# ducha-aiki/affnet

Measured on NVIDIA H100. Metric: Mpix/s end-to-end HesAffNet(+OriNet)+HardNet, higher is better.
Workload: dtype fp16 operands (fp16 residual planes: AffNet/OriNet weights+activations, HardNet layer 2-3 weights), fp32 accumulate; stencils fp32

## Files before the change

affnet_b200/_lib.py:

```python
import ctypes as C
import os
import subprocess

import torch

HERE = os.path.dirname(os.path.abspath(__file__))
LIB_PATH = os.environ.get("AFFNET_B200_LIB", os.path.join(HERE, "lib", "libaffnet_b200.so"))
AG_MAX_OCTAVES, AG_MAX_LEVELS = 16, 8
NET_AFFNET, NET_ORINET, NET_HARDNET = 0, 1, 2
ENGINE_SIMT, ENGINE_TC, ENGINE_TC_EXACT, ENGINE_TC_FAST, ENGINE_TC2, ENGINE_TC2_BF16 = 0, 1, 2, 3, 4, 5


class AffnetB200Error(RuntimeError):
    pass


class PyramidPlan(C.Structure):
    _fields_ = [
        ("B", C.c_int), ("H", C.c_int), ("W", C.c_int), ("n_octaves", C.c_int), ("n_levels", C.c_int),
        ("h", C.c_int * AG_MAX_OCTAVES), ("w", C.c_int * AG_MAX_OCTAVES),
        ("level_offset", (C.c_longlong * AG_MAX_LEVELS) * AG_MAX_OCTAVES),
        ("total_floats", C.c_longlong),
        ("sigma", (C.c_double * AG_MAX_LEVELS) * AG_MAX_OCTAVES),
        ("blur_sigma", (C.c_double * AG_MAX_LEVELS) * AG_MAX_OCTAVES),
# ... 48 lines not shown
    "ag_detect_ws_carve": (i32, [C.POINTER(PyramidPlan), i32, vp, C.POINTER(DetectWs)]),
    "ag_detect": (i32, [C.POINTER(PyramidPlan), vp, f32, i32, C.POINTER(DetectWs), vp]),
    "ag_detect_level_from_responses": (i32, [vp, vp, vp, i32, i32, C.POINTER(f64), i32, vp, vp, i32, C.POINTER(DetectWs), vp]),
    "ag_select_keypoints": (i32, [C.POINTER(PyramidPlan), C.POINTER(DetectWs), i32, f32, i32, vp, vp, vp, vp, vp, vp]),
    "ag_select_all_workspace_bytes": (sz, [C.POINTER(PyramidPlan), i32]),
    "ag_select_all_keypoints": (i32, [C.POINTER(PyramidPlan), C.POINTER(DetectWs), f32, i32, vp, sz, vp, vp, vp, vp, vp, vp]),
    "ag_select_topk_workspace_bytes": (sz, [C.POINTER(PyramidPlan), i32, i32]),
    "ag_select_topk_keypoints": (i32, [C.POINTER(PyramidPlan), C.POINTER(DetectWs), i32, f32, i32, vp, sz, vp, vp, vp, vp, vp, vp]),
    "ag_extract_patches": (i32, [vp, i32, i32, i32, i32, vp, i32, i32, vp, vp]),
    "ag_extract_patches_pyr": (i32, [C.POINTER(PyramidPlan), vp, vp, vp, vp, vp, i32, i32, vp, vp]),
    "ag_pyramid_level_for_lafs": (i32, [C.POINTER(PyramidPlan), vp, i32, i32, vp, vp, vp]),
    "ag_net_create": (i32, [i32, vp, sz, C.POINTER(vp)]),
    "ag_net_destroy": (None, [vp]),
    "ag_net_blob_floats": (sz, [i32]),
    "ag_net_set_engine": (i32, [vp, i32]),
    "ag_net_get_engine": (i32, [vp]),
    "ag_net_workspace_bytes": (sz, [i32, i32]),
    "ag_mat2_compose": (i32, [vp, vp, vp, i32, vp]),
    "ag_lafs_left_multiply": (i32, [vp, vp, vp, i32, vp]),
    "ag_affnet_forward_raw": (i32, [vp, vp, i32, vp, vp, sz, vp]),
    "ag_orinet_forward_raw": (i32, [vp, vp, i32, vp, vp, sz, vp]),
    "ag_debug_pyramid_mode": (i32, [i32]),
    "ag_debug_tcx_layer": (i32, [vp, vp, i32, i32, vp, vp, sz, vp]),
    "ag_debug_libm": (i32, [vp, vp, i32, vp, vp, vp, vp]),
    "ag_debug_orientation_hist_pyr": (i32, [C.POINTER(PyramidPlan), vp, vp, vp, vp, vp, i32, i32, vp, vp, vp]),
    "ag_debug_baumberg_pyr": (i32, [C.POINTER(PyramidPlan), vp, vp, vp, vp, vp, i32, i32, i32, vp, vp, vp]),
    "ag_affnet_forward": (i32, [vp, vp, i32, vp, i32, vp, vp, sz, vp]),
    "ag_orinet_forward": (i32, [vp, vp, i32, vp, i32, vp, vp, vp, sz, vp]),
    "ag_hardnet_forward": (i32, [vp, vp, i32, vp, i32, vp, vp, sz, vp]),
    "ag_net_forward_pyr": (i32, [vp, C.POINTER(PyramidPlan), vp, vp, vp, vp, vp, i32, vp, vp, sz, vp]),
    "ag_affine_shape_filter": (i32, [vp, vp, vp, vp, vp, vp, i32, i32, i32, i32, vp, vp, vp, vp, vp, vp]),
    "ag_affine_shape_filter_all": (i32, [vp, vp, vp, vp, vp, vp, i32, i32, vp, vp, vp, vp, vp, vp]),
    "ag_affine_shape_filter_topk_workspace_bytes": (sz, [i32, i32]),
    "ag_affine_shape_filter_topk": (i32, [vp, vp, vp, vp, vp, vp, i32, i32, i32, i32, vp, sz, vp, vp, vp, vp, vp, vp]),
    "ag_lafs_apply_rotation": (i32, [vp, vp, i32, vp]),
    "ag_lafs_scale": (i32, [vp, vp, i32, f32, f32, f32, vp]),
    "ag_lafs_to_ell": (i32, [vp, i32, vp, vp]),
    "ag_circular_gauss_kernel": (i32, [i32, f64, vp]),
    "ag_orientation_hist": (i32, [vp, i32, i32, vp, vp, vp]),
    "ag_baumberg_shape": (i32, [vp, i32, i32, vp, vp, vp]),
    "ag_sift_windows": (i32, [i32, vp, vp, C.POINTER(i32), C.POINTER(i32)]),
    "ag_sift_describe": (i32, [vp, i32, i32, f32, vp, vp]),
    "ag_sift_describe_pyr": (i32, [C.POINTER(PyramidPlan), vp, vp, vp, vp, vp, i32, i32, f32, vp, vp]),
    "ag_distance_matrix": (i32, [vp, i32, vp, i32, i32, vp, vp]),
    "ag_match_snn_workspace_bytes": (sz, [i32, i32]),
    "ag_match_snn": (i32, [vp, i32, vp, i32, i32, f32, vp, sz, vp, vp, vp, vp, vp]),
# ... 94 lines not shown
```

affnet_b200/csrc/net_impl.cuh:

```cuda
#pragma once
#include <cuda_fp16.h>

#include <vector>

#include "common.cuh"

#define AG_ENGINE_SIMT 0
#define AG_ENGINE_TC 1
#define AG_ENGINE_TC_EXACT 2
#define AG_ENGINE_TC2 4
#define AG_ENGINE_TC2_BF16 5
#define AG_ENGINE_TC_FAST 3

struct ag_net {
    int kind;
    int engine;
    float* d_w[6];
    float* d_b[6];
    float* d_w1;
    __half* d_wx[6];
    __half* d_all_x;
    __half* d_wx_bf[6];
    __half* d_headh_bf;
    __half* d_wh[6];
// ... 8 lines not shown
};

#include "tc_conv.cuh"

namespace ag {
size_t tc_act_bytes(int kind);
int tc_nsplit(int kind, int layer);
int tc_split_w(int kind);
tc::FirstSrc tc_src_patches(const float* patches);
tc::FirstSrc tc_src_pyramid(const ag_pyramid_plan_t* p, const float* pyr, const float* lafs, const int* oct, const int* lvl, int cap);
int tc_hardnet_forward(const ag_net* net, const tc::FirstSrc& src, int n, int group, const int* count, void* bufA, void* bufB, void* headbuf,
                       float* out, cudaStream_t st);
int tc_trunk_orinet(const ag_net* net, const tc::FirstSrc& src, int n, int group, const int* count, void* bufA, void* bufB, void* feat,
                    cudaStream_t st);
int tc_trunk_affnet(const ag_net* net, const tc::FirstSrc& src, int n, int group, const int* count, void* bufA, void* bufB, void* feat,
                    cudaStream_t st);
int tc_headx_forward(const ag_net* net, const void* feat, int n, int group, const int* count, float* out, float* angle, cudaStream_t st, float* raw = nullptr);
size_t tc_headx_bytes(int n);
void tcx_pack_layer(const float* wf, int ci, int co, int stride, int nsplit, int sw, float scale, std::vector<__half>& out, int bf16 = 0);
int tcx_nsplit(int kind, int layer);
int tcx_split_w(int kind, int layer);
int tcx_stride(int layer);
size_t tcx_act_bytes(int n);
int tcx_trunk_affori(const ag_net* net, const tc::FirstSrc& src, int n, int group, const int* count, void* bufA, void* bufB, void* feat,
                     cudaStream_t st, int upto);
int tcx_trunk_hardnet(const ag_net* net, const tc::FirstSrc& src, int n, int group, const int* count, void* bufA, void* bufB, void* headbuf,
                      cudaStream_t st, int upto, int bf16 = 0);
int tc_hardnet_head(const ag_net* net, const void* headbuf, int n, int group, const int* count, float* out, cudaStream_t st, int bf16 = 0);
}
```

affnet_b200/csrc/nets_simt.cu:

```cuda
#include <math.h>

#include <vector>

#include <cuda_bf16.h>

#include "net_impl.cuh"

namespace ag {

constexpr float BN_EPS = 1e-5f;
constexpr int CNT = 256;

struct LayerCfg {
    int cin, cout, stride, hin;
};
static const LayerCfg kAffCfg[6] = {{1, 16, 1, 32}, {16, 16, 1, 32}, {16, 32, 2, 32}, {32, 32, 1, 16}, {32, 64, 2, 16}, {64, 64, 1, 8}};
static const LayerCfg kHardCfg[6] = {{1, 32, 1, 32}, {32, 32, 1, 32}, {32, 64, 2, 32}, {64, 64, 1, 16}, {64, 128, 2, 16}, {128, 128, 1, 8}};

}

namespace ag {

template <int CIN, int COUT, int HIN, int STRIDE, int CT, int CK, bool NORM>
__global__ void __launch_bounds__(CNT) conv3x3_kernel(const float* __restrict__ in, float* __restrict__ out,
// ... 507 lines not shown
    if ((rc = launch_conv<32, 32, 32, 1, 32, 32, false>(a, b, net->d_w[1], net->d_b[1], n, group, count, st))) return rc;
    if ((rc = launch_conv<32, 64, 32, 2, 64, 32, false>(b, a, net->d_w[2], net->d_b[2], n, group, count, st))) return rc;
    if ((rc = launch_conv<64, 64, 16, 1, 64, 32, false>(a, b, net->d_w[3], net->d_b[3], n, group, count, st))) return rc;
    if ((rc = launch_conv<64, 128, 16, 2, 128, 16, false>(b, a, net->d_w[4], net->d_b[4], n, group, count, st))) return rc;
    if ((rc = launch_conv<128, 128, 8, 1, 128, 16, false>(a, b, net->d_w[5], net->d_b[5], n, group, count, st))) return rc;
    return AG_OK;
}

static int run_trunk(const ag_net* net, const float* patches, const tc::FirstSrc* pyr_src, int n, int group, const int* count, float* a,
                     float* b, float** feat, cudaStream_t st) {
    if (net->engine != AG_ENGINE_SIMT) {
        const tc::FirstSrc src = pyr_src ? *pyr_src : tc_src_patches(patches);
        char* base = (char*)a;
        const size_t total = 2 * (size_t)((char*)b - (char*)a);
        const size_t act = net->engine == AG_ENGINE_TC2 ? align_up(tcx_act_bytes(n), 256)
                                                        : align_up((size_t)n * tc_act_bytes(net->engine == AG_ENGINE_TC_FAST ? net->kind : AG_NET_ORINET), 256);
        const size_t fbytes = tc_headx_bytes(n);
        if (2 * act + fbytes > total) { set_error("tensor-core workspace too small"); return AG_ERR_CAPACITY; }
        void* bufA = base;
        void* bufB = base + act;
        b = (float*)(base + 2 * act);
        *feat = b;
        if (net->kind == AG_NET_HARDNET) { set_error("HardNet tensor-core path has its own entry"); return AG_ERR_INVALID; }
        if (net->engine == AG_ENGINE_TC2) return tcx_trunk_affori(net, src, n, group, count, bufA, bufB, b, st, 6);
        if (net->engine != AG_ENGINE_TC_FAST) return tc_trunk_orinet(net, src, n, group, count, bufA, bufB, b, st);
        return tc_trunk_affnet(net, src, n, group, count, bufA, bufB, b, st);
    }
    *feat = b;
    if (patches == nullptr) { set_error("the fp32 SIMT engine needs materialised patches"); return AG_ERR_INVALID; }
    return net->kind == AG_NET_HARDNET ? trunk_hardnet(net, patches, n, group, count, a, b, st)
                                       : trunk_affnet(net, patches, n, group, count, a, b, st);
}

static int split_ws(int kind, int n, void* d_ws, size_t ws_bytes, float** a, float** b) {
    const size_t need = ag_net_workspace_bytes(kind, n);
    if (d_ws == nullptr || ws_bytes < need) {
        set_error("net forward: workspace of %zu bytes needed, %zu given", need, ws_bytes);
        return AG_ERR_CAPACITY;
    }
    *a = (float*)d_ws;
    *b = (float*)((char*)d_ws + need / 2);
    return AG_OK;
}

}

extern "C" {
// ... 105 lines not shown
```

affnet_b200/csrc/nets_tcx.cu:

```cuda
#include <stdlib.h>
#include <string.h>

#include <vector>

#include <cuda_bf16.h>

#include "net_impl.cuh"
#include "tcx_conv.cuh"
#include "tcx_first.cuh"

namespace ag {
namespace tcx {

static int num_sms() {
    static int n = 0;
    if (n == 0) {
        int dev = 0;
        cudaGetDevice(&dev);
        cudaDeviceGetAttribute(&n, cudaDevAttrMultiProcessorCount, dev);
        if (n <= 0) n = 132;
    }
    return n;
}

static int ensure_smem_attr(const void* func, int bytes, bool* configured, const char* what) {
    int dev = 0;
    cudaGetDevice(&dev);
    dev &= 63;
    if (configured[dev]) return AG_OK;
    int rc = check_cuda(cudaFuncSetAttribute(func, cudaFuncAttributeMaxDynamicSharedMemorySize, bytes), what);
    if (rc == AG_OK) configured[dev] = true;
    return rc;
// ... 4 lines not shown
    using Cfg = XCfg<CIN, COUT, H, STRIDE, NSPLIT, STAGES, OUT, SA, SW, OSA>;
    auto kern = tcx_conv_kernel<CIN, COUT, H, STRIDE, NSPLIT, STAGES, OUT, SA, SW, OSA, BF, MC, PPS>;
    static bool configured[64] = {};
    int rc = ensure_smem_attr((const void*)kern, (int)Cfg::SMEM, configured, "tcx_conv smem attr");
    if (rc != AG_OK) return rc;
    XArgs a;
    a.in = (const __half*)in; a.out = out; a.wpk = w; a.bias = b; a.inv_scale = inv_scale; a.n = n; a.group = group; a.count = count;
    const int units = Cfg::In::PAIR ? (n + 1) / 2 : n;
    int gx = num_sms() / NSPLIT;
    if (gx > units) gx = units;
    if (gx < 1) gx = 1;
    if (MC) {
        cudaLaunchConfig_t cfg;
        memset(&cfg, 0, sizeof(cfg));
        cfg.gridDim = dim3(gx, NSPLIT); cfg.blockDim = dim3(Cfg::THREADS); cfg.dynamicSmemBytes = Cfg::SMEM; cfg.stream = st;
        cudaLaunchAttribute attr[1];
        attr[0].id = cudaLaunchAttributeClusterDimension;
        attr[0].val.clusterDim.x = 1; attr[0].val.clusterDim.y = 2; attr[0].val.clusterDim.z = 1;
        cfg.attrs = attr; cfg.numAttrs = 1;
        rc = check_cuda(cudaLaunchKernelEx(&cfg, kern, a), "tcx_conv cluster launch");
        if (rc != AG_OK) return rc;
    } else
        kern<<<dim3(gx, NSPLIT), Cfg::THREADS, Cfg::SMEM, st>>>(a);
    AG_CHECK_LAUNCH("tcx_conv_kernel");
    return AG_OK;
}

template <int C1, int COUT, int SA, int SW, int OSA, int BF = 0, int L3 = 0>
static int launch_first(void* out, const __half* w, const float* b, float inv_scale, int n, int group, const int* count, cudaStream_t st, const FirstSrc& src,
                        void* out3 = nullptr, const __half* w3 = nullptr, const float* b3 = nullptr, float inv_scale3 = 0.f) {
    using Cfg = XFirstCfg<C1, COUT, SA, SW, OSA, L3>;
    auto kern = tcx_first_kernel<C1, COUT, SA, SW, OSA, BF, L3>;
    static bool configured[64] = {};
    int rc = ensure_smem_attr((const void*)kern, (int)Cfg::SMEM, configured, "tcx_first smem attr");
    if (rc != AG_OK) return rc;
    XArgs a;
    a.in = nullptr; a.out = out; a.wpk = w; a.bias = b; a.inv_scale = inv_scale; a.n = n; a.group = group; a.count = count;
    XArgs a3 = a;
    a3.out = out3; a3.wpk = w3; a3.bias = b3; a3.inv_scale = inv_scale3;
    int gx = num_sms();
    if (gx > n) gx = n;
    if (gx < 1) gx = 1;
    kern<<<gx, Cfg::THREADS, Cfg::SMEM, st>>>(a, src, a3);
    AG_CHECK_LAUNCH("tcx_first_kernel");
    return AG_OK;
}
// ... 69 lines not shown

int tcx_nsplit(int kind, int layer) { return (kind == AG_NET_HARDNET && layer >= 4) ? 2 : 1; }
#ifndef AG_HARD_SW2
#define AG_HARD_SW2 1
#endif
#ifndef AG_HARD_SW3
#define AG_HARD_SW3 1
#endif
#ifndef AG_HARD_SW4
#define AG_HARD_SW4 0
#endif
int tcx_split_w(int kind, int layer) { return kind == AG_NET_HARDNET ? (layer == 1 ? AG_HARD_SW2 : layer == 2 ? AG_HARD_SW3 : layer == 3 ? AG_HARD_SW4 : 0) : 1; }
int tcx_stride(int layer) { return (layer == 2 || layer == 4) ? 2 : 1; }

size_t tcx_act_bytes(int n) { return (size_t)(n + 1) * 65536; }

#ifndef AG_HARD_MC5
#define AG_HARD_MC5 1
#endif
#ifndef AG_HARD_MC6
#define AG_HARD_MC6 0
#endif
int tcx_trunk_affori(const ag_net* net, const tc::FirstSrc& src0, int n, int group, const int* count, void* bufA, void* bufB, void* feat,
                     cudaStream_t st, int upto) {
    using namespace tcx;
    tc::FirstSrc src = src0;
    src.w1 = net->d_w1; src.b1 = net->d_b[0]; src.w1_inv = net->w_inv_scale[0]; src.w1_scale = 1.0f / net->w_inv_scale[0];
    int rc;
    if (upto <= 2) return launch_first<16, 16, 1, 1, 1>(bufB, net->d_wx[1], net->d_b[1], net->w_inv_scale[1], n, group, count, st, src);
    if ((rc = launch_first<16, 16, 1, 1, 1, 0, 1>(nullptr, net->d_wx[1], net->d_b[1], net->w_inv_scale[1], n, group, count, st, src,
                                                   bufA, net->d_wx[2], net->d_b[2], net->w_inv_scale[2]))) return rc;
    if (upto <= 3) return AG_OK;
    if ((rc = launch_conv<32, 32, 16, 1, 1, 4, L_S2_8P, 1, 1, 1>(bufA, bufB, net->d_wx[3], net->d_b[3], net->w_inv_scale[3], n, group, count, st))) return rc;
    if (upto <= 4) return AG_OK;
    if ((rc = launch_conv<32, 64, 16, 2, 1, 2, L_S1_8P, 1, 1, 1>(bufB, bufA, net->d_wx[4], net->d_b[4], net->w_inv_scale[4], n, group, count, st))) return rc;
    if (upto <= 5) return AG_OK;
    return launch_conv<64, 64, 8, 1, 1, 2, L_HEAD, 1, 1, 1, 0, 0, 1>(bufA, feat, net->d_wx[5], net->d_b[5], net->w_inv_scale[5], n, group, count, st);
}

template <int BF>
static int trunk_hardnet_t(const ag_net* net, const tc::FirstSrc& src0, int n, int group, const int* count, void* bufA, void* bufB, void* headbuf,
                           cudaStream_t st, int upto) {
    using namespace tcx;
    tc::FirstSrc src = src0;
    src.w1 = net->d_w1; src.b1 = net->d_b[0]; src.w1_inv = net->w_inv_scale[0]; src.w1_scale = 1.0f / net->w_inv_scale[0];
    __half* const* wx = BF ? net->d_wx_bf : net->d_wx;
    int rc;
    if ((rc = launch_first<32, 32, 0, AG_HARD_SW2, 0, BF>(bufB, wx[1], net->d_b[1], net->w_inv_scale[1], n, group, count, st, src))) return rc;
    if (upto <= 2) return AG_OK;
    if ((rc = launch_conv<32, 64, 32, 2, 1, 2, L_S1_16, 0, AG_HARD_SW3, 0, BF>(bufB, bufA, wx[2], net->d_b[2], net->w_inv_scale[2], n, group, count, st))) return rc;
    if (upto <= 3) return AG_OK;
    if ((rc = launch_conv<64, 64, 16, 1, 1, 2, L_S2_8P, 0, AG_HARD_SW4, 0, BF>(bufA, bufB, wx[3], net->d_b[3], net->w_inv_scale[3], n, group, count, st))) return rc;
    if (upto <= 4) return AG_OK;
    if ((rc = launch_conv<64, 128, 16, 2, 2, 2, L_S1_8P, 0, 0, 0, BF, AG_HARD_MC5, 1>(bufB, bufA, wx[4], net->d_b[4], net->w_inv_scale[4], n, group, count, st))) return rc;
    if (upto <= 5) return AG_OK;
    return launch_conv<128, 128, 8, 1, 2, 2, L_HEAD, 0, 0, 0, BF, AG_HARD_MC6, 1>(bufA, headbuf, wx[5], net->d_b[5], net->w_inv_scale[5], n, group, count, st);
}

int tcx_trunk_hardnet(const ag_net* net, const tc::FirstSrc& src0, int n, int group, const int* count, void* bufA, void* bufB, void* headbuf,
                      cudaStream_t st, int upto, int bf16) {
    return bf16 ? trunk_hardnet_t<1>(net, src0, n, group, count, bufA, bufB, headbuf, st, upto)
                : trunk_hardnet_t<0>(net, src0, n, group, count, bufA, bufB, headbuf, st, upto);
}

}

using namespace ag;

extern "C" {

int ag_debug_tcx_layer(const ag_net_t* net, const float* d_patches, int n, int upto, float* d_out, void* d_ws, size_t ws_bytes, void* stream) {
    AG_REQUIRE(net && d_patches && d_out && d_ws, "NULL argument");
    AG_REQUIRE(upto >= 2 && upto <= 6 && n >= 1, "layer out of range");
    const size_t act = align_up(tcx_act_bytes(n), 256);
    AG_REQUIRE(ws_bytes >= ag_net_workspace_bytes(net->kind, n), "workspace too small");
    cudaStream_t st = (cudaStream_t)stream;
    char* base = (char*)d_ws;
    const tc::FirstSrc src = tc_src_patches(d_patches);
    const bool hard = net->kind == AG_NET_HARDNET;
    const int bf = hard && net->engine == AG_ENGINE_TC2_BF16;
    int rc = hard ? tcx_trunk_hardnet(net, src, n, n, nullptr, base, base + act, base + 2 * act, st, upto, bf)
                  : tcx_trunk_affori(net, src, n, n, nullptr, base, base + act, base + 2 * act, st, upto);
    if (rc) return rc;
    const int lay = upto == 2 ? tcx::L_S2_16 : upto == 3 ? tcx::L_S1_16 : upto == 4 ? tcx::L_S2_8P : upto == 5 ? tcx::L_S1_8P : tcx::L_HEAD;
    const int H = upto == 2 ? 32 : (upto <= 4 ? 16 : 8);
    const int Cb = hard ? 32 : 16;
    const int C = upto == 2 ? Cb : (upto <= 4 ? 2 * Cb : 4 * Cb);
    const void* buf = upto == 6 ? base + 2 * act : (upto == 2 || upto == 4) ? base + act : base;
    const int osa = hard ? 0 : 1;
    tcx::tcx_decode_kernel<<<296, 256, 0, st>>>((const __half*)buf, lay, C, osa, H, n, bf, d_out);
    AG_CHECK_LAUNCH("tcx_decode_kernel");
    return AG_OK;
}

#ifdef AG_FIRST_TIMELINE
int ag_first_timeline_read(unsigned long long* host, int* dims, int reset) {
    constexpr size_t n = (size_t)tcx::TL_LAUNCHES * tcx::TL_CTAS * 16 * tcx::TL_STATES;
    if (dims) { dims[0] = tcx::TL_LAUNCHES; dims[1] = tcx::TL_CTAS; dims[2] = tcx::TL_STATES; }
    cudaDeviceSynchronize();
    if (host) {
        const int rc = check_cuda(cudaMemcpyFromSymbol(host, tcx::g_first_tl, n * 8), "timeline read");
        if (rc != AG_OK) return rc;
    }
    if (reset) {
        static unsigned long long zeros[n];
        static int zl[tcx::TL_CTAS];
        int rc = check_cuda(cudaMemcpyToSymbol(tcx::g_first_tl, zeros, sizeof(zeros)), "timeline reset");
        if (rc == AG_OK) rc = check_cuda(cudaMemcpyToSymbol(tcx::g_first_tl_launch, zl, sizeof(zl)), "timeline reset");
        return rc;
    }
    return AG_OK;
}
#endif
// ... 24 lines not shown
```

affnet_b200/csrc/tcx_conv.cuh:

```cuda
#pragma once
#include <cuda_bf16.h>

#include "tc_conv.cuh"

#ifndef AG_CONV_PINGPONG
#define AG_CONV_PINGPONG 1
#endif

namespace ag {
namespace tcx {

using namespace ag::tc;

constexpr int XORDER = 5;

enum { CT_TOTAL, CT_WAIT_FULL, CT_TURN, CT_ISSUE, CT_MMA_WAIT, CT_EPILOGUE, CT_WG_BAR, CT_WAIT_EMPTY, CT_OTHER, CT_STATES };
#ifdef AG_CONV_TIMELINE
constexpr int CT_CTAS = 4, CT_LAUNCHES = 16, CT_EVENTS = 2048;
__device__ unsigned long long g_conv_tl[CT_LAUNCHES][CT_CTAS][9][CT_STATES];
__device__ unsigned long long g_conv_ev[CT_LAUNCHES][2][CT_EVENTS][3];
__device__ int g_conv_tl_launch[CT_CTAS];
struct ConvTimeline {
    unsigned long long t[CT_STATES];
    long long start, mark;
    int slot, warp, n_ev;
    __device__ static void claim(int* s_slot) {
        if (threadIdx.x == 0)
            *s_slot = (blockIdx.y == 0 && blockIdx.x < CT_CTAS) ? min(atomicAdd(&g_conv_tl_launch[blockIdx.x], 1), CT_LAUNCHES) : CT_LAUNCHES;
    }
    __device__ void init(const int* s_slot) {
        for (int i = 0; i < CT_STATES; i++) t[i] = 0;
        slot = *s_slot; warp = threadIdx.x >> 5; n_ev = 0;
        start = mark = clock64();
    }
    __device__ void lap(int state) { const long long now = clock64(); t[state] += (unsigned long long)(now - mark); mark = now; }
    __device__ void event(int k) {
        if (blockIdx.x == 0 && slot < CT_LAUNCHES && (threadIdx.x & 127) == 0 && n_ev < CT_EVENTS) g_conv_ev[slot][warp >> 2][n_ev][k] = (unsigned long long)mark;
        if (k == 2) n_ev++;
    }
    __device__ void finish() {
        t[CT_TOTAL] = (unsigned long long)(clock64() - start);
        if ((threadIdx.x & 31) == 0 && slot < CT_LAUNCHES)
            for (int i = 0; i < CT_STATES; i++) g_conv_tl[slot][blockIdx.x][warp][i] = t[i];
    }
};
#else
struct ConvTimeline {
    __device__ static void claim(int*) {}
    __device__ void init(const int*) {}
    __device__ void lap(int) {}
    __device__ void event(int) {}
    __device__ void finish() {}
};
#endif

enum XLayout { L_S2_16 = 0, L_S1_16 = 1, L_S2_8P = 2, L_S1_8P = 3, L_HEAD = 4 };

__device__ __forceinline__ void bulk_g2s_mc(void* dst, const void* src, uint32_t bytes, uint64_t* bar, uint16_t mask) {
    asm volatile("cp.async.bulk.shared::cluster.global.mbarrier::complete_tx::bytes.multicast::cluster [%0], [%1], %2, [%3], %4;" ::"r"(smem_u32(dst)),
                 "l"(src), "r"(bytes), "r"(smem_u32(bar)), "h"(mask)
                 : "memory");
}
__device__ __forceinline__ void mbar_arrive_cluster(uint64_t* bar, uint32_t cta) {
    asm volatile("{\n .reg .b32 ra;\n mapa.shared::cluster.u32 ra, %0, %1;\n mbarrier.arrive.release.cta.shared::cluster.b64 _, [ra];\n}\n" ::"r"(smem_u32(bar)), "r"(cta)
                 : "memory");
}
__device__ __forceinline__ void cluster_sync() {
    asm volatile("barrier.cluster.arrive.release.aligned;\n barrier.cluster.wait.acquire.aligned;" ::: "memory");
}

template <int BF>
__device__ __forceinline__ uint32_t pack2(float a, float b) {
    if (BF) { const __nv_bfloat162 h = __floats2bfloat162_rn(a, b); return *reinterpret_cast<const uint32_t*>(&h); }
    const __half2 h = __floats2half2_rn(a, b);
// ... 124 lines not shown
            constexpr int PL = In::PLANE;
            const int py = (dy == 1) ? 0 : 1, ro = (dy == 0) ? 0 : 1;
#pragma unroll
            for (int j = 0; j < KC / 2; j++) {
                const uint32_t blk = w_base + (uint32_t)((dy * (KC / 2) + j) * 2 * (Cfg::NRO + Cfg::NRE));
                const uint32_t bo_hi = (blk & 0x3FFFu) | ((uint32_t)Cfg::NRO << 16), bo_lo = ((blk + 2 * NT) & 0x3FFFu) | ((uint32_t)Cfg::NRO << 16);
                const uint32_t be = blk + 2 * Cfg::NRO;
                const uint32_t be_hi = (be & 0x3FFFu) | ((uint32_t)Cfg::NRE << 16), be_lo = ((be + NT) & 0x3FFFu) | ((uint32_t)Cfg::NRE << 16);
                const uint32_t ao = a_t + (uint32_t)((py * 2 + 1) * PL + ro * RW);
                const uint32_t ao_hi = ((ao + (uint32_t)(2 * j * GS)) & 0x3FFFu) | LBO_A, ao_lo = ((ao + (uint32_t)((KC + 2 * j) * GS)) & 0x3FFFu) | LBO_A;
                Wgmma<2 * NT, BF>::mma(d, desc64(ao_hi), desc64(bo_hi), (dy | j) != 0);
                if (SW) Wgmma<2 * NT, BF>::mma(d, desc64(ao_hi), desc64(bo_lo), 1);
                if (SA) Wgmma<2 * NT, BF>::mma(d, desc64(ao_lo), desc64(bo_hi), 1);
                const uint32_t ae = a_t + (uint32_t)((py * 2 + 0) * PL + ro * RW);
                const uint32_t ae_hi = ((ae + (uint32_t)(2 * j * GS)) & 0x3FFFu) | LBO_A, ae_lo = ((ae + (uint32_t)((KC + 2 * j) * GS)) & 0x3FFFu) | LBO_A;
                Wgmma<NT, BF>::mma(d + NT, desc64(ae_hi), desc64(be_hi), (dy | j) != 0);
                if (SW) Wgmma<NT, BF>::mma(d + NT, desc64(ae_hi), desc64(be_lo), 1);
                if (SA) Wgmma<NT, BF>::mma(d + NT, desc64(ae_lo), desc64(be_hi), 1);
            }
        }
    }
    wgmma_commit();
}
template <class Cfg, int BF>
__device__ __forceinline__ void xconv_block_epilogue(const float* d, const XArgs& a, const float* s_bias, int u, int b, int split, int wq, int lane) {
    using In = typename Cfg::In;
    constexpr int NT = Cfg::NT, HOUT = Cfg::HOUT, W = In::W, PAIR = In::PAIR, COUT = Cfg::CO, OUT = Cfg::OUTL, OSA = Cfg::SPLIT_O;
    unsigned char* obase[2];
    bool ok[2];
    size_t lo_off = 0;
    const int i = lane >> 2, xi = PAIR ? (i & 3) : i;
    const bool has_l0 = xi > 0, has_r1 = xi < W / 2 - 1;
    static_assert(W == 16 || PAIR, "neighbour-paired row groups: 16 pixels, or 8 of each patch of a pair");
#pragma unroll
    for (int h = 0; h < 2; h++) {
        const int y = b * 4 + wq, x = 2 * xi + h, pi = PAIR ? 2 * u + (i >> 2) : u;
        ok[h] = xpatch_valid(a, pi);
        if (OUT == L_HEAD) {
            obase[h] = reinterpret_cast<unsigned char*>(a.out) + (((size_t)(pi >> 7) * (HOUT * HOUT * COUT / 8) + (size_t)(y * HOUT + x) * (COUT / 8)) * 128 + (pi & 127)) * 16;
            lo_off = (size_t)((a.n + 127) >> 7) * (HOUT * HOUT * COUT / 8) * 128 * 16;
        } else {
            const int ou = layout_pair(OUT) ? (pi >> 1) : pi;
            obase[h] = reinterpret_cast<unsigned char*>(a.out) + (size_t)ou * Cfg::UNIT_OUT_BYTES + (size_t)layout_slot(OUT, y, x, pi & 1) * 16;
            lo_off = (size_t)(COUT / 8) * layout_slots(OUT) * 16;
        }
    }
#pragma unroll
    for (int j = 0; j < NT / 8; j++) {
        const int c = j * 8 + 2 * (lane & 3);
        float v[2][2];
#pragma unroll
        for (int e = 0; e < 2; e++) {
            const float c00 = d[4 * j + e], c01 = d[4 * j + 2 + e];
            const float c10 = d[4 * (j + NT / 8) + e], c11 = d[4 * (j + NT / 8) + 2 + e];
            const float c20 = d[4 * (j + 2 * NT / 8) + e], c21 = d[4 * (j + 2 * NT / 8) + 2 + e];
            const float l0 = frag_left_even(c01, lane);
            float acc0, acc1;
            if (Cfg::STRD == 1) {
                const float r1 = frag_right_odd(c20, lane);
                const float t0 = c21 + c10, t1 = has_r1 ? r1 + c11 : c11;
                acc0 = has_l0 ? l0 + t0 : t0;
                acc1 = c00 + t1;
            } else {
                const float t0 = c10 + c20, t1 = c11 + c21;
                acc0 = has_l0 ? l0 + t0 : t0;
                acc1 = c00 + t1;
            }
            v[0][e] = fmaxf(fmaf(acc0, a.inv_scale, s_bias[c + e]), 0.f);
            v[1][e] = fmaxf(fmaf(acc1, a.inv_scale, s_bias[c + e]), 0.f);
        }
        const int ch = split * NT + c;
        const size_t goff = ((OUT == L_HEAD) ? (size_t)(ch / 8) * 128 * 16 : (size_t)(ch / 8) * layout_slots(OUT) * 16) + (ch & 7) * 2;
#pragma unroll
        for (int h = 0; h < 2; h++) {
            if (!ok[h]) continue;
            uint32_t hi, lo;
            split_pack2<OSA, BF>(v[h][0], v[h][1], hi, lo);
            *reinterpret_cast<uint32_t*>(obase[h] + goff) = hi;
            if (OSA) *reinterpret_cast<uint32_t*>(obase[h] + lo_off + goff) = lo;
        }
    }
}

template <int CIN, int COUT, int H, int STRIDE, int NSPLIT, int STAGES, int OUT, int SA, int SW, int OSA, int BF = 0, int MC = 0, int PPS = 0>
__global__ void __launch_bounds__(288, 1) tcx_conv_kernel(const XArgs a) {
    static_assert(MC == 0 || NSPLIT == 2, "multicast pairs the two channel-split CTAs");
    using Cfg = XCfg<CIN, COUT, H, STRIDE, NSPLIT, STAGES, OUT, SA, SW, OSA>;
    using In = typename Cfg::In;
    constexpr int ACCW = Cfg::ACCW, BLOCKS = Cfg::BLOCKS, GS = Cfg::GS, RW = In::RW;
    constexpr int PAIR = In::PAIR;
    constexpr bool PP = AG_CONV_PINGPONG && PPS;
    extern __shared__ __align__(1024) unsigned char smem[];
    uint64_t* full = reinterpret_cast<uint64_t*>(smem);
    uint64_t* empty = full + STAGES;
    uint64_t* wbar = empty + STAGES;
// ... 109 lines not shown
```

include/affnet_b200.h:

```cpp
#ifndef AFFNET_B200_H
#define AFFNET_B200_H

#include <stddef.h>
#include <stdint.h>

#ifdef __cplusplus
extern "C" {
#endif

#define AG_OK 0
#define AG_ERR_INVALID -1
#define AG_ERR_CUDA -2
#define AG_ERR_CAPACITY -3
#define AG_ERR_NO_DEVICE -4

#define AG_MAX_OCTAVES 16
#define AG_MAX_LEVELS 8

const char* ag_last_error(void);
int ag_abi_version(void);

int ag_prof_begin(void* stream);
int ag_prof_end(void);
int ag_prof_get(int i, const char** name, float* ms);
// ... 58 lines not shown

int ag_extract_patches(const float* d_img, int C, int h, int w, int per_patch_img, const float* d_lafs, int n,
                       int PS, float* d_out, void* stream);

int ag_extract_patches_pyr(const ag_pyramid_plan_t* plan, const float* d_pyr, const float* d_lafs, const int* d_oct,
                           const int* d_lvl, const int* d_count, int cap, int PS, float* d_out, void* stream);

int ag_pyramid_level_for_lafs(const ag_pyramid_plan_t* plan, const float* d_dlafs, int n, int PS, int* d_oct,
                              int* d_lvl, void* stream);

#define AG_NET_AFFNET 0
#define AG_NET_ORINET 1
#define AG_NET_HARDNET 2

typedef struct ag_net ag_net_t;

int ag_net_create(int kind, const float* h_blob, size_t n_floats, ag_net_t** out);
void ag_net_destroy(ag_net_t* net);
size_t ag_net_blob_floats(int kind);
int ag_net_set_engine(ag_net_t* net, int engine);
int ag_net_get_engine(const ag_net_t* net);
int ag_debug_pyramid_mode(int fused);
int ag_debug_tcx_layer(const ag_net_t* net, const float* d_patches, int n, int upto, float* d_out, void* d_ws, size_t ws_bytes, void* stream);
int ag_debug_libm(const float* d_y, const float* d_x, int n, float* d_atan2, float* d_cos, float* d_sin, void* stream);
int ag_debug_orientation_hist_pyr(const ag_pyramid_plan_t* plan, const float* d_pyr, const float* d_lafs, const int* d_oct, const int* d_lvl,
                                  const int* d_count, int cap, int PS, const float* h_gk, float* d_R, void* stream);
int ag_debug_baumberg_pyr(const ag_pyramid_plan_t* plan, const float* d_pyr, const float* d_lafs, const int* d_oct, const int* d_lvl,
                          const int* d_count, int cap, int PS, int iters, const float* h_gk, float* d_A, void* stream);
size_t ag_net_workspace_bytes(int kind, int n);

int ag_affnet_forward(const ag_net_t* net, const float* d_patches, int n, const int* d_count, int group, float* d_out,
                      void* d_ws, size_t ws_bytes, void* stream);
int ag_orinet_forward(const ag_net_t* net, const float* d_patches, int n, const int* d_count, int group, float* d_out,
                      float* d_angle, void* d_ws, size_t ws_bytes, void* stream);
int ag_hardnet_forward(const ag_net_t* net, const float* d_patches, int n, const int* d_count, int group, float* d_out,
                       void* d_ws, size_t ws_bytes, void* stream);

int ag_affnet_forward_raw(const ag_net_t* net, const float* d_patches, int n, float* d_raw, void* d_ws, size_t ws_bytes, void* stream);
int ag_orinet_forward_raw(const ag_net_t* net, const float* d_patches, int n, float* d_raw, void* d_ws, size_t ws_bytes, void* stream);
int ag_net_forward_pyr(const ag_net_t* net, const ag_pyramid_plan_t* plan, const float* d_pyr, const float* d_lafs, const int* d_oct,
                       const int* d_lvl, const int* d_count, int cap, float* d_out, void* d_ws, size_t ws_bytes, void* stream);

int ag_affine_shape_filter(const float* d_A, const float* d_resp, const float* d_lafs, const int* d_oct,
                           const int* d_lvl, const int* d_count_in, int B, int cap, int num_features, int out_cap,
                           float* d_resp_out, float* d_lafs_out, int* d_oct_out, int* d_lvl_out, int* d_count_out,
                           void* stream);
// ... 97 lines not shown
```

Measured before the change: 682.4.

## Fuse AffNet/OriNet conv layers 4 and 5 into one persistent wgmma kernel

Adds a persistent kernel that computes trunk layer 4 for a pair of patches and writes its output straight into shared memory in the layout layer 5 reads, then runs layer 5 from smem. This removes one launch and the global-memory round trip of the layer-4 activations for AffNet/OriNet on the TC2 engine. It is enabled by default through a compile-time flag and changes which buffer holds the layer-5 output. In exchange it uses fewer pipeline stages and serialises layer 5 behind both layer-4 patches, which can lower overlap. A debug entry point is added to compare the fused and unfused paths.

```diff
diff --git a/affnet_b200/_lib.py b/affnet_b200/_lib.py
--- a/affnet_b200/_lib.py
+++ b/affnet_b200/_lib.py
@@ -94,6 +94,7 @@
     "ag_orinet_forward_raw": (i32, [vp, vp, i32, vp, vp, sz, vp]),
     "ag_debug_pyramid_mode": (i32, [i32]),
     "ag_debug_tcx_layer": (i32, [vp, vp, i32, i32, vp, vp, sz, vp]),
+    "ag_debug_tcx_l5": (i32, [vp, vp, i32, i32, vp, i32, vp, vp, sz, vp]),
     "ag_debug_libm": (i32, [vp, vp, i32, vp, vp, vp, vp]),
     "ag_debug_orientation_hist_pyr": (i32, [C.POINTER(PyramidPlan), vp, vp, vp, vp, vp, i32, i32, vp, vp, vp]),
     "ag_debug_baumberg_pyr": (i32, [C.POINTER(PyramidPlan), vp, vp, vp, vp, vp, i32, i32, i32, vp, vp, vp]),
diff --git a/affnet_b200/csrc/net_impl.cuh b/affnet_b200/csrc/net_impl.cuh
--- a/affnet_b200/csrc/net_impl.cuh
+++ b/affnet_b200/csrc/net_impl.cuh
@@ -54,8 +54,11 @@
 int tcx_split_w(int kind, int layer);
 int tcx_stride(int layer);
 size_t tcx_act_bytes(int n);
+#ifndef AG_AFFORI_FUSE45
+#define AG_AFFORI_FUSE45 1
+#endif
 int tcx_trunk_affori(const ag_net* net, const tc::FirstSrc& src, int n, int group, const int* count, void* bufA, void* bufB, void* feat,
-                     cudaStream_t st, int upto);
+                     cudaStream_t st, int upto, int fuse45);
 int tcx_trunk_hardnet(const ag_net* net, const tc::FirstSrc& src, int n, int group, const int* count, void* bufA, void* bufB, void* headbuf,
                       cudaStream_t st, int upto, int bf16 = 0);
 int tc_hardnet_head(const ag_net* net, const void* headbuf, int n, int group, const int* count, float* out, cudaStream_t st, int bf16 = 0);
diff --git a/affnet_b200/csrc/nets_simt.cu b/affnet_b200/csrc/nets_simt.cu
--- a/affnet_b200/csrc/nets_simt.cu
+++ b/affnet_b200/csrc/nets_simt.cu
@@ -553,7 +553,7 @@
         b = (float*)(base + 2 * act);
         *feat = b;
         if (net->kind == AG_NET_HARDNET) { set_error("HardNet tensor-core path has its own entry"); return AG_ERR_INVALID; }
-        if (net->engine == AG_ENGINE_TC2) return tcx_trunk_affori(net, src, n, group, count, bufA, bufB, b, st, 6);
+        if (net->engine == AG_ENGINE_TC2) return tcx_trunk_affori(net, src, n, group, count, bufA, bufB, b, st, 6, AG_AFFORI_FUSE45);
         if (net->engine != AG_ENGINE_TC_FAST) return tc_trunk_orinet(net, src, n, group, count, bufA, bufB, b, st);
         return tc_trunk_affnet(net, src, n, group, count, bufA, bufB, b, st);
     }
diff --git a/affnet_b200/csrc/nets_tcx.cu b/affnet_b200/csrc/nets_tcx.cu
--- a/affnet_b200/csrc/nets_tcx.cu
+++ b/affnet_b200/csrc/nets_tcx.cu
@@ -8,6 +8,7 @@
 #include "net_impl.cuh"
 #include "tcx_conv.cuh"
 #include "tcx_first.cuh"
+#include "tcx_l45.cuh"
 
 namespace ag {
 namespace tcx {
@@ -58,6 +59,27 @@
         if (rc != AG_OK) return rc;
     } else
         kern<<<dim3(gx, NSPLIT), Cfg::THREADS, Cfg::SMEM, st>>>(a);
+    AG_CHECK_LAUNCH("tcx_conv_kernel");
+    return AG_OK;
+}
+
+using XL4 = XCfg<32, 32, 16, 1, 1, 1, L_S2_8P, 1, 1, 1>;
+using XL5 = XCfg<32, 64, 16, 2, 1, 1, L_S1_8P, 1, 1, 1>;
+static int launch_l45(const void* in, void* out, const __half* w4, const float* b4, float inv4, const __half* w5, const float* b5, float inv5, int n,
+                      int group, const int* count, cudaStream_t st) {
+    using Cfg = XL45Cfg<XL4, XL5>;
+    auto kern = tcx_l45_kernel<XL4, XL5>;
+    static bool configured[64] = {};
+    int rc = ensure_smem_attr((const void*)kern, (int)Cfg::SMEM, configured, "tcx_l45 smem attr");
+    if (rc != AG_OK) return rc;
+    XArgs a4, a5;
+    a4.in = (const __half*)in; a4.out = nullptr; a4.wpk = w4; a4.bias = b4; a4.inv_scale = inv4; a4.n = n; a4.group = group; a4.count = count;
+    a5 = a4;
+    a5.in = nullptr; a5.out = out; a5.wpk = w5; a5.bias = b5; a5.inv_scale = inv5;
+    int gx = num_sms();
+    if (gx > (n + 1) / 2) gx = (n + 1) / 2;
+    if (gx < 1) gx = 1;
+    kern<<<gx, Cfg::THREADS, Cfg::SMEM, st>>>(a4, a5);
     AG_CHECK_LAUNCH("tcx_conv_kernel");
     return AG_OK;
 }
@@ -173,7 +195,7 @@
 #define AG_HARD_MC6 0
 #endif
 int tcx_trunk_affori(const ag_net* net, const tc::FirstSrc& src0, int n, int group, const int* count, void* bufA, void* bufB, void* feat,
-                     cudaStream_t st, int upto) {
+                     cudaStream_t st, int upto, int fuse45) {
     using namespace tcx;
     tc::FirstSrc src = src0;
     src.w1 = net->d_w1; src.b1 = net->d_b[0]; src.w1_inv = net->w_inv_scale[0]; src.w1_scale = 1.0f / net->w_inv_scale[0];
@@ -182,11 +204,18 @@
     if ((rc = launch_first<16, 16, 1, 1, 1, 0, 1>(nullptr, net->d_wx[1], net->d_b[1], net->w_inv_scale[1], n, group, count, st, src,
                                                    bufA, net->d_wx[2], net->d_b[2], net->w_inv_scale[2]))) return rc;
     if (upto <= 3) return AG_OK;
-    if ((rc = launch_conv<32, 32, 16, 1, 1, 4, L_S2_8P, 1, 1, 1>(bufA, bufB, net->d_wx[3], net->d_b[3], net->w_inv_scale[3], n, group, count, st))) return rc;
-    if (upto <= 4) return AG_OK;
-    if ((rc = launch_conv<32, 64, 16, 2, 1, 2, L_S1_8P, 1, 1, 1>(bufB, bufA, net->d_wx[4], net->d_b[4], net->w_inv_scale[4], n, group, count, st))) return rc;
+    const bool fused = upto >= 5 && fuse45;
+    void* const l5out = fused ? bufB : bufA;
+    if (fused) {
+        if ((rc = launch_l45(bufA, l5out, net->d_wx[3], net->d_b[3], net->w_inv_scale[3], net->d_wx[4], net->d_b[4], net->w_inv_scale[4], n, group, count, st)))
+            return rc;
+    } else {
+        if ((rc = launch_conv<32, 32, 16, 1, 1, 4, L_S2_8P, 1, 1, 1>(bufA, bufB, net->d_wx[3], net->d_b[3], net->w_inv_scale[3], n, group, count, st))) return rc;
+        if (upto <= 4) return AG_OK;
+        if ((rc = launch_conv<32, 64, 16, 2, 1, 2, L_S1_8P, 1, 1, 1>(bufB, bufA, net->d_wx[4], net->d_b[4], net->w_inv_scale[4], n, group, count, st))) return rc;
+    }
     if (upto <= 5) return AG_OK;
-    return launch_conv<64, 64, 8, 1, 1, 2, L_HEAD, 1, 1, 1, 0, 0, 1>(bufA, feat, net->d_wx[5], net->d_b[5], net->w_inv_scale[5], n, group, count, st);
+    return launch_conv<64, 64, 8, 1, 1, 2, L_HEAD, 1, 1, 1, 0, 0, 1>(l5out, feat, net->d_wx[5], net->d_b[5], net->w_inv_scale[5], n, group, count, st);
 }
 
 template <int BF>
@@ -231,15 +260,31 @@
     const bool hard = net->kind == AG_NET_HARDNET;
     const int bf = hard && net->engine == AG_ENGINE_TC2_BF16;
     int rc = hard ? tcx_trunk_hardnet(net, src, n, n, nullptr, base, base + act, base + 2 * act, st, upto, bf)
-                  : tcx_trunk_affori(net, src, n, n, nullptr, base, base + act, base + 2 * act, st, upto);
+                  : tcx_trunk_affori(net, src, n, n, nullptr, base, base + act, base + 2 * act, st, upto, AG_AFFORI_FUSE45);
     if (rc) return rc;
     const int lay = upto == 2 ? tcx::L_S2_16 : upto == 3 ? tcx::L_S1_16 : upto == 4 ? tcx::L_S2_8P : upto == 5 ? tcx::L_S1_8P : tcx::L_HEAD;
     const int H = upto == 2 ? 32 : (upto <= 4 ? 16 : 8);
     const int Cb = hard ? 32 : 16;
     const int C = upto == 2 ? Cb : (upto <= 4 ? 2 * Cb : 4 * Cb);
-    const void* buf = upto == 6 ? base + 2 * act : (upto == 2 || upto == 4) ? base + act : base;
+    const void* buf = upto == 6 ? base + 2 * act : (upto == 2 || upto == 4 || (upto == 5 && !hard && AG_AFFORI_FUSE45)) ? base + act : base;
     const int osa = hard ? 0 : 1;
     tcx::tcx_decode_kernel<<<296, 256, 0, st>>>((const __half*)buf, lay, C, osa, H, n, bf, d_out);
+    AG_CHECK_LAUNCH("tcx_decode_kernel");
+    return AG_OK;
+}
+
+int ag_debug_tcx_l5(const ag_net_t* net, const float* d_patches, int n, int group, const int* d_count, int fused, float* d_out, void* d_ws,
+                    size_t ws_bytes, void* stream) {
+    AG_REQUIRE(net && d_patches && d_out && d_ws, "NULL argument");
+    AG_REQUIRE(net->kind != AG_NET_HARDNET, "AffNet / OriNet only");
+    AG_REQUIRE(n >= 1 && group >= 1 && n % group == 0, "bad patch count or group");
+    AG_REQUIRE(ws_bytes >= ag_net_workspace_bytes(net->kind, n), "workspace too small");
+    const size_t act = align_up(tcx_act_bytes(n), 256);
+    cudaStream_t st = (cudaStream_t)stream;
+    char* base = (char*)d_ws;
+    int rc = tcx_trunk_affori(net, tc_src_patches(d_patches), n, group, d_count, base, base + act, base + 2 * act, st, 5, fused);
+    if (rc) return rc;
+    tcx::tcx_decode_kernel<<<296, 256, 0, st>>>((const __half*)(fused ? base + act : base), tcx::L_S1_8P, 64, 1, 8, n, 0, d_out);
     AG_CHECK_LAUNCH("tcx_decode_kernel");
     return AG_OK;
 }
diff --git a/affnet_b200/csrc/tcx_conv.cuh b/affnet_b200/csrc/tcx_conv.cuh
--- a/affnet_b200/csrc/tcx_conv.cuh
+++ b/affnet_b200/csrc/tcx_conv.cuh
@@ -1,5 +1,7 @@
 #pragma once
 #include <cuda_bf16.h>
+
+#include <type_traits>
 
 #include "tc_conv.cuh"
 
@@ -34,10 +36,12 @@
         start = mark = clock64();
     }
     __device__ void lap(int state) { const long long now = clock64(); t[state] += (unsigned long long)(now - mark); mark = now; }
-    __device__ void event(int k) {
-        if (blockIdx.x == 0 && slot < CT_LAUNCHES && (threadIdx.x & 127) == 0 && n_ev < CT_EVENTS) g_conv_ev[slot][warp >> 2][n_ev][k] = (unsigned long long)mark;
+    __device__ void event(int k) { event(k, mark); }
+    __device__ void event(int k, long long at) {
+        if (blockIdx.x == 0 && slot < CT_LAUNCHES && (threadIdx.x & 127) == 0 && n_ev < CT_EVENTS) g_conv_ev[slot][warp >> 2][n_ev][k] = (unsigned long long)at;
         if (k == 2) n_ev++;
     }
+    __device__ long long stamp() const { return mark; }
     __device__ void finish() {
         t[CT_TOTAL] = (unsigned long long)(clock64() - start);
         if ((threadIdx.x & 31) == 0 && slot < CT_LAUNCHES)
@@ -50,6 +54,8 @@
     __device__ void init(const int*) {}
     __device__ void lap(int) {}
     __device__ void event(int) {}
+    __device__ void event(int, long long) {}
+    __device__ long long stamp() const { return 0; }
     __device__ void finish() {}
 };
 #endif
@@ -220,8 +226,9 @@
     }
     wgmma_commit();
 }
-template <class Cfg, int BF>
-__device__ __forceinline__ void xconv_block_epilogue(const float* d, const XArgs& a, const float* s_bias, int u, int b, int split, int wq, int lane) {
+template <class Cfg, int BF, class Dst = void>
+__device__ __forceinline__ void xconv_block_epilogue(const float* d, const XArgs& a, const float* s_bias, int u, int b, int split, int wq, int lane,
+                                                     unsigned char* stage = nullptr) {
     using In = typename Cfg::In;
     constexpr int NT = Cfg::NT, HOUT = Cfg::HOUT, W = In::W, PAIR = In::PAIR, COUT = Cfg::CO, OUT = Cfg::OUTL, OSA = Cfg::SPLIT_O;
     unsigned char* obase[2];
@@ -234,7 +241,13 @@
     for (int h = 0; h < 2; h++) {
         const int y = b * 4 + wq, x = 2 * xi + h, pi = PAIR ? 2 * u + (i >> 2) : u;
         ok[h] = xpatch_valid(a, pi);
-        if (OUT == L_HEAD) {
+        if constexpr (!std::is_void<Dst>::value) {
+            using DIn = typename Dst::In;
+            static_assert(DIn::LAYOUT == OUT && Dst::KC == COUT / 8 && Dst::SPLIT_A == OSA, "the next layer reads this layer's output");
+            const int sl = layout_slot(OUT, y, x, pi & 1);
+            obase[h] = stage + ((size_t)(sl / DIn::DATA) * DIn::PLANE + DIn::RW + sl % DIn::DATA) * 16;
+            lo_off = (size_t)(COUT / 8) * Dst::GS * 16;
+        } else if (OUT == L_HEAD) {
             obase[h] = reinterpret_cast<unsigned char*>(a.out) + (((size_t)(pi >> 7) * (HOUT * HOUT * COUT / 8) + (size_t)(y * HOUT + x) * (COUT / 8)) * 128 + (pi & 127)) * 16;
             lo_off = (size_t)((a.n + 127) >> 7) * (HOUT * HOUT * COUT / 8) * 128 * 16;
         } else {
@@ -268,7 +281,9 @@
             v[1][e] = fmaxf(fmaf(acc1, a.inv_scale, s_bias[c + e]), 0.f);
         }
         const int ch = split * NT + c;
-        const size_t goff = ((OUT == L_HEAD) ? (size_t)(ch / 8) * 128 * 16 : (size_t)(ch / 8) * layout_slots(OUT) * 16) + (ch & 7) * 2;
+        size_t goff;
+        if constexpr (!std::is_void<Dst>::value) goff = (size_t)(ch / 8) * Dst::GS * 16 + (ch & 7) * 2;
+        else goff = ((OUT == L_HEAD) ? (size_t)(ch / 8) * 128 * 16 : (size_t)(ch / 8) * layout_slots(OUT) * 16) + (ch & 7) * 2;
 #pragma unroll
         for (int h = 0; h < 2; h++) {
             if (!ok[h]) continue;
diff --git a/affnet_b200/csrc/tcx_l45.cuh b/affnet_b200/csrc/tcx_l45.cuh
--- /dev/null
+++ b/affnet_b200/csrc/tcx_l45.cuh
@@ -0,0 +1,153 @@
+#pragma once
+#include "tcx_conv.cuh"
+
+namespace ag {
+namespace tcx {
+
+template <class C4, class C5>
+struct XL45Cfg {
+    static constexpr size_t SMEM = 1024 + (size_t)C4::W_BYTES + C5::W_BYTES + C4::IN_BYTES + C5::IN_BYTES;
+    static constexpr int THREADS = 288;
+    static_assert(C4::STRD == 1 && !C4::In::PAIR && C5::In::PAIR, "layer 4 of single patches feeds layer 5 of pairs");
+    static_assert(C4::GS == C4::In::SLOT_STAGE + C4::In::RW && C5::GS == C5::In::SLOT_STAGE, "one stage of each layer");
+    static_assert(C4::NT == C4::CO && C5::NT == C5::CO, "no channel split");
+    static_assert(C4::BLOCKS == 4 && C5::BLOCKS == 2, "two layer-4 blocks and one layer-5 block per warpgroup");
+    static_assert(C4::NT <= 32 && C5::NT <= 96, "biases fit smem[512, 1024)");
+    static_assert(SMEM <= 232448, "shared memory budget");
+};
+
+template <class C4, class C5, int BF = 0>
+__global__ void __launch_bounds__(288, 1) tcx_l45_kernel(const XArgs a4, const XArgs a5) {
+    using Cfg = XL45Cfg<C4, C5>;
+    using In4 = typename C4::In;
+    constexpr bool PP = AG_CONV_PINGPONG;
+    extern __shared__ __align__(1024) unsigned char smem[];
+    uint64_t* full = reinterpret_cast<uint64_t*>(smem);
+    uint64_t* empty = full + 1;
+    uint64_t* free5 = full + 2;
+    uint64_t* wbar = full + 3;
+    int* s_tl_slot = reinterpret_cast<int*>(smem + 496);
+    float* s_bias4 = reinterpret_cast<float*>(smem + 512);
+    float* s_bias5 = reinterpret_cast<float*>(smem + 640);
+    unsigned char* sW4 = smem + 1024;
+    unsigned char* sW5 = sW4 + C4::W_BYTES;
+    unsigned char* sIn4 = sW5 + C5::W_BYTES;
+    unsigned char* sIn5 = sIn4 + C4::IN_BYTES;
+
+    const int warp = threadIdx.x >> 5, lane = threadIdx.x & 31;
+    const int n_units = (a4.n + 1) >> 1;
+
+    if (threadIdx.x < C4::NT) s_bias4[threadIdx.x] = a4.bias[threadIdx.x];
+    if (threadIdx.x < C5::NT) s_bias5[threadIdx.x] = a5.bias[threadIdx.x];
+    if (threadIdx.x == 0) {
+        mbar_init(full, 1); mbar_init(empty, 8); mbar_init(free5, 8); mbar_init(wbar, 1);
+        asm volatile("fence.mbarrier_init.release.cluster;" ::: "memory");
+    }
+    ConvTimeline::claim(s_tl_slot);
+    for (int i = threadIdx.x; i < (int)((C4::IN_BYTES + C5::IN_BYTES) / 16); i += blockDim.x) reinterpret_cast<uint4*>(sIn4)[i] = make_uint4(0, 0, 0, 0);
+    asm volatile("fence.proxy.async.shared::cta;" ::: "memory");
+    __syncthreads();
+    ConvTimeline tl;
+    tl.init(s_tl_slot);
+
+    if (warp == 8) {
+        if (lane == 0) {
+            mbar_expect_tx(wbar, C4::W_BYTES + C5::W_BYTES);
+            bulk_g2s(sW4, a4.wpk, C4::W_BYTES, wbar);
+            bulk_g2s(sW5, a5.wpk, C5::W_BYTES, wbar);
+            int it = 0;
+            for (int u = blockIdx.x; u < n_units; u += gridDim.x) {
+#pragma unroll 1
+                for (int p = 0; p < 2; p++) {
+                    const int pi = 2 * u + p;
+                    if (!xpatch_valid(a4, pi)) continue;
+                    const unsigned char* gsrc = reinterpret_cast<const unsigned char*>(a4.in) + (size_t)pi * C4::UNIT_IN_BYTES;
+                    if (p == 0 && xpatch_valid(a4, pi + 1))
+                        asm volatile("cp.async.bulk.prefetch.L2.global [%0], %1;" ::"l"(gsrc + C4::UNIT_IN_BYTES), "r"(C4::UNIT_IN_BYTES) : "memory");
+                    tl.lap(CT_OTHER);
+                    mbar_wait(empty, (it & 1) ^ 1);
+                    tl.lap(CT_WAIT_EMPTY);
+                    mbar_expect_tx(full, C4::UNIT_IN_BYTES);
+#pragma unroll 1
+                    for (int g = 0; g < C4::G; g++)
+                        bulk_g2s(sIn4 + ((size_t)g * C4::GS + In4::RW) * 16, gsrc + (size_t)g * In4::DATA * 16, In4::DATA * 16u, full);
+                    it++;
+                }
+            }
+            tl.lap(CT_OTHER);
+        }
+    } else if (warp < 8) {
+        const int wg = warp >> 2, wq = warp & 3;
+        mbar_wait(wbar, 0);
+        const uint32_t w4_base = smem_u32(sW4) >> 4, w5_base = smem_u32(sW5) >> 4;
+        const uint32_t in4_base = smem_u32(sIn4) >> 4, in5_base = smem_u32(sIn5) >> 4;
+        int it = 0, k = 0;
+        for (int u = blockIdx.x; u < n_units; u += gridDim.x) {
+            const bool v0 = xpatch_valid(a4, 2 * u), v1 = xpatch_valid(a4, 2 * u + 1);
+            if (!v0 && !v1) continue;
+#pragma unroll 1
+            for (int p = v0 ? 0 : 1; p < (v1 ? 2 : 1); p++) {
+                const int pi = 2 * u + p;
+                tl.lap(CT_OTHER);
+                mbar_wait(full, it & 1);
+                tl.lap(CT_WAIT_FULL);
+                if (PP && (wg == 1 || it > 0)) bar_sync(XORDER + wg, 256);
+                tl.lap(CT_TURN);
+                const long long t_issue = tl.stamp();
+                float d[2][C4::ACCW / 2];
+                xconv_block_issue<C4, BF>(d[0], in4_base + (uint32_t)(wg * 64), w4_base);
+                xconv_block_issue<C4, BF>(d[1], in4_base + (uint32_t)((wg + 2) * 64), w4_base);
+                if (PP) asm volatile("bar.arrive %0, 256;" ::"r"(XORDER + (wg ^ 1)) : "memory");
+                tl.lap(CT_ISSUE);
+                if (p == (v0 ? 0 : 1) && k > 0) {
+                    mbar_wait(free5, (k - 1) & 1);
+                    tl.lap(CT_TURN);
+                }
+                wgmma_wait<1>();
+                wgmma_reg_fence<C4::ACCW / 2>(d[0]);
+                tl.lap(CT_MMA_WAIT);
+                const long long t_done0 = tl.stamp();
+                tl.event(0, t_issue);
+                tl.event(1);
+                xconv_block_epilogue<C4, BF, C5>(d[0], a4, s_bias4, pi, wg, 0, wq, lane, sIn5);
+                tl.lap(CT_EPILOGUE);
+                tl.event(2);
+                wgmma_wait<0>();
+                wgmma_reg_fence<C4::ACCW / 2>(d[1]);
+                tl.lap(CT_MMA_WAIT);
+                if (lane == 0) mbar_arrive(empty);
+                tl.event(0, t_done0);
+                tl.event(1);
+                xconv_block_epilogue<C4, BF, C5>(d[1], a4, s_bias4, pi, wg + 2, 0, wq, lane, sIn5);
+                tl.lap(CT_EPILOGUE);
+                tl.event(2);
+                it++;
+            }
+            asm volatile("fence.proxy.async.shared::cta;" ::: "memory");
+            bar_sync(3, 256);
+            tl.lap(CT_WG_BAR);
+            if (PP) bar_sync(XORDER + wg, 256);
+            tl.lap(CT_TURN);
+            tl.event(0);
+            float d5[C5::ACCW / 2];
+            xconv_block_issue<C5, BF>(d5, in5_base + (uint32_t)(wg * 64), w5_base);
+            if (PP) asm volatile("bar.arrive %0, 256;" ::"r"(XORDER + (wg ^ 1)) : "memory");
+            tl.lap(CT_ISSUE);
+            wgmma_wait<0>();
+            wgmma_reg_fence<C5::ACCW / 2>(d5);
+            tl.lap(CT_MMA_WAIT);
+            tl.event(1);
+            if (lane == 0) mbar_arrive(free5);
+            xconv_block_epilogue<C5, BF>(d5, a5, s_bias5, u, wg, 0, wq, lane);
+            tl.lap(CT_EPILOGUE);
+            tl.event(2);
+            k++;
+        }
+        if (PP && wg == 0 && it > 0) bar_sync(XORDER, 256);
+        tl.lap(CT_OTHER);
+    }
+    tl.finish();
+}
+
+}
+}
diff --git a/include/affnet_b200.h b/include/affnet_b200.h
--- a/include/affnet_b200.h
+++ b/include/affnet_b200.h
@@ -104,6 +104,8 @@
 int ag_net_get_engine(const ag_net_t* net);
 int ag_debug_pyramid_mode(int fused);
 int ag_debug_tcx_layer(const ag_net_t* net, const float* d_patches, int n, int upto, float* d_out, void* d_ws, size_t ws_bytes, void* stream);
+int ag_debug_tcx_l5(const ag_net_t* net, const float* d_patches, int n, int group, const int* d_count, int fused, float* d_out, void* d_ws,
+                    size_t ws_bytes, void* stream);
 int ag_debug_libm(const float* d_y, const float* d_x, int n, float* d_atan2, float* d_cos, float* d_sin, void* stream);
 int ag_debug_orientation_hist_pyr(const ag_pyramid_plan_t* plan, const float* d_pyr, const float* d_lafs, const int* d_oct, const int* d_lvl,
                                   const int* d_count, int cap, int PS, const float* h_gk, float* d_R, void* stream);
```

Result: faster. 692.6 (median of 6 runs) (+1.5%).
